# intel/oim

Hardware: AMD Instinct MI355X
Metric: 4KiB_randread_IOPS (higher is better)
Workload: dtype uint8

## Files before the change

### native/src/gpu.hip

```cpp

#include <hip/hip_runtime.h>
#include <pthread.h>
#include <sched.h>
#include <unistd.h>
#include <stdlib.h>

#include <algorithm>
#include <atomic>
#include <chrono>
#include <condition_variable>
#include <cstring>
#include <deque>
#include <functional>
#include <map>
#include <mutex>
#include <random>
#include <set>
#include <stdexcept>
#include <thread>
#include <utility>
#include <vector>

#include "hipstore/crc32c.h"
#include "hipstore/engine.h"
// ... 187 lines not shown
       w += gridDim.x) {
    const unsigned long long word = bitmap[w];
    const uint64_t g0 = w * 64;
    unsigned long long inside = word;
    if (g0 < win.g_begin) inside &= ~0ull << (win.g_begin - g0);
    if (win.g_end - g0 < 64) inside &= (1ull << (win.g_end - g0)) - 1;
    uint32_t bits = __builtin_amdgcn_readfirstlane(static_cast<uint32_t>(
        (inside >> (wave * kDiffGranulesPerWave)) & 0xFFFFu));
    if (bits == 0) continue;
    const uint32_t rank0 =
        __builtin_amdgcn_readfirstlane(rank_before_word[w]) - win.first_rank;
    while (bits != 0) {
      const uint32_t bit = wave * kDiffGranulesPerWave +
                           static_cast<uint32_t>(__builtin_ctz(bits));
      bits &= bits - 1;
      const uint32_t slot =
          rank0 + static_cast<uint32_t>(__popcll(word & ((1ull << bit) - 1)));
      if (slot >= win.count) break;
      uint4* __restrict__ pg = reinterpret_cast<uint4*>(
          bdev_base + (g0 + bit) * granule_bytes);
      uint4* __restrict__ ps = reinterpret_cast<uint4*>(
          dense + static_cast<uint64_t>(slot) * granule_bytes);
      if (kPack) {
#pragma unroll 4
        for (uint32_t i = lane; i < n16; i += 64) ps[i] = pg[i];
      } else {
#pragma unroll 4
        for (uint32_t i = lane; i < n16; i += 64) pg[i] = ps[i];
      }
    }
  }
}

__global__ __launch_bounds__(kWavesPerWg * 64) void k_pack_marked(
    const uint8_t* __restrict__ src, uint8_t* __restrict__ dense,
    const unsigned long long* __restrict__ bitmap,
    const uint32_t* __restrict__ rank_before_word, MarkedWindow win,
    uint32_t granule_bytes) {
  marked_window_walk<true>(const_cast<uint8_t*>(src), dense, bitmap,
                           rank_before_word, win, granule_bytes);
}

__global__ __launch_bounds__(kWavesPerWg * 64) void k_unpack_marked(
    uint8_t* __restrict__ dst, const uint8_t* __restrict__ dense,
    const unsigned long long* __restrict__ bitmap,
    const uint32_t* __restrict__ rank_before_word, MarkedWindow win,
    uint32_t granule_bytes) {
  marked_window_walk<false>(dst, const_cast<uint8_t*>(dense), bitmap,
                            rank_before_word, win, granule_bytes);
}


__device__ __forceinline__ unsigned long long wave_bcast_u64(
    unsigned long long v) {
  int lo = __shfl(static_cast<int>(v & 0xFFFFFFFFu), 0);
  int hi = __shfl(static_cast<int>(v >> 32), 0);
  return (static_cast<unsigned long long>(static_cast<uint32_t>(hi)) << 32) |
         static_cast<uint32_t>(lo);
}

__device__ __forceinline__ unsigned long long claim_bounded(
    unsigned long long* counter, unsigned long long c,
    unsigned long long kt, uint32_t lane) {
  while (c < kt) {
    unsigned long long witnessed = 0;
    if (lane == 0) {
      witnessed = atomicCAS(counter, c, c + 1);
    }
    witnessed = wave_bcast_u64(witnessed);
    if (witnessed == c) return c;
    c = witnessed;
  }
  return ~0ull;
}

struct PersistentCtl {
  const BlockDesc* sq;
  volatile unsigned long long* sq_tail;
  volatile unsigned long long* cq;
  volatile uint32_t* stop;
  unsigned long long* claim_counter;
  unsigned long long* known_tail;
  uint32_t* exit_flag;
  uint32_t ring_mask;
  uint32_t idle_spins;
};

__global__ __launch_bounds__(64) void k_persistent_copy(PersistentCtl ctl) {
  __shared__ __attribute__((aligned(16))) uint8_t lds_raw[kTileBytes];
  const uint32_t lane = threadIdx.x & 63;
  float4* lds = reinterpret_cast<float4*>(lds_raw);

  if (blockIdx.x == 0) {
    if (lane != 0) return;
    unsigned long long known = __hip_atomic_load(
        ctl.known_tail, __ATOMIC_RELAXED, __HIP_MEMORY_SCOPE_AGENT);
    uint32_t spins = 0;
    while (true) {
      unsigned long long tail = __hip_atomic_load(
          const_cast<const unsigned long long*>(ctl.sq_tail),
          __ATOMIC_ACQUIRE, __HIP_MEMORY_SCOPE_SYSTEM);
      if (tail > known) {
        known = tail;
        __hip_atomic_store(ctl.known_tail, known, __ATOMIC_RELEASE,
                           __HIP_MEMORY_SCOPE_AGENT);
        spins = 0;
      }
      if (__hip_atomic_load(const_cast<const uint32_t*>(ctl.stop),
                            __ATOMIC_RELAXED,
                            __HIP_MEMORY_SCOPE_SYSTEM) != 0 ||
          ++spins > ctl.idle_spins) {
        __hip_atomic_store(ctl.exit_flag, 1u, __ATOMIC_RELEASE,
                           __HIP_MEMORY_SCOPE_AGENT);
        return;
      }
      __builtin_amdgcn_s_sleep(8);
    }
  }

  while (true) {
    const unsigned long long kt = __hip_atomic_load(
        ctl.known_tail, __ATOMIC_RELAXED, __HIP_MEMORY_SCOPE_AGENT);
    const unsigned long long c = __hip_atomic_load(
        ctl.claim_counter, __ATOMIC_RELAXED, __HIP_MEMORY_SCOPE_AGENT);
    const unsigned long long claim =
        claim_bounded(ctl.claim_counter, c, kt, lane);
    if (claim == ~0ull) {
      if (__hip_atomic_load(ctl.exit_flag, __ATOMIC_RELAXED,
                            __HIP_MEMORY_SCOPE_AGENT) != 0) {
        return;
      }
      __builtin_amdgcn_s_sleep(16);
      continue;
    }
    const volatile unsigned long long* vd =
        reinterpret_cast<const volatile unsigned long long*>(
            &ctl.sq[claim & ctl.ring_mask]);
    const unsigned long long w0 = vd[0];
    const unsigned long long w1 = vd[1];
    const unsigned long long w2 = vd[2];
    BlockDesc d;
    d.src = reinterpret_cast<const uint8_t*>(w0);
    d.dst = reinterpret_cast<uint8_t*>(w1);
    d.bytes = static_cast<uint32_t>(w2 & 0xFFFFFFFFu);
    d.fill = static_cast<uint32_t>(w2 >> 32);
    const uint32_t n8 = d.bytes >> 3;
    unsigned long long* lds64 = reinterpret_cast<unsigned long long*>(lds);
    if (d.src != nullptr) {
      const unsigned long long* __restrict__ src =
          reinterpret_cast<const unsigned long long*>(d.src);
#pragma unroll 4
      for (uint32_t i = lane; i < n8; i += 64) {
        lds64[i] = __hip_atomic_load(src + i, __ATOMIC_RELAXED,
                                     __HIP_MEMORY_SCOPE_AGENT);
      }
    } else {
      const uint32_t b = d.fill & 0xFF;
      const uint32_t word = b | (b << 8) | (b << 16) | (b << 24);
      const unsigned long long v =
          word | (static_cast<unsigned long long>(word) << 32);
      for (uint32_t i = lane; i < n8; i += 64) lds64[i] = v;
    }
    unsigned long long* __restrict__ dst =
        reinterpret_cast<unsigned long long*>(d.dst);
#pragma unroll 4
    for (uint32_t i = lane; i < n8; i += 64) dst[i] = lds64[i];
    if (lane == 0) {
      __hip_atomic_store(&ctl.cq[claim & ctl.ring_mask], claim + 1,
                         __ATOMIC_RELEASE, __HIP_MEMORY_SCOPE_SYSTEM);
    }
  }
}

__global__ void k_init_ctl(unsigned long long* dst, unsigned long long a,
                           unsigned long long b, unsigned long long c) {
  if (threadIdx.x == 0) {
    dst[0] = a;
    dst[1] = b;
    dst[2] = c;
  }
}

std::atomic<uint64_t> g_pers_launches{0};
std::atomic<uint64_t> g_pers_relaunches{0};
std::atomic<uint64_t> g_pers_stall_queries{0};


struct SharedSlot {
  const BlockDesc* sq;
  volatile unsigned long long* sq_tail;
  volatile unsigned long long* cq;
  unsigned long long claim;
  unsigned long long known_tail;
  unsigned long long ring_mask_active;
};
static_assert(sizeof(SharedSlot) == 48, "8-byte atom layout");

constexpr uint32_t kSharedSlots = 64;

struct SharedCtl {
  SharedSlot* slots;
  volatile uint32_t* stop;
  uint32_t* exit_flag;
  uint32_t idle_spins;
};

__device__ __forceinline__ unsigned long long slot_ld(
    SharedSlot* slot, int word) {
  return __hip_atomic_load(
      reinterpret_cast<unsigned long long*>(slot) + word, __ATOMIC_RELAXED,
      __HIP_MEMORY_SCOPE_AGENT);
}

__device__ __forceinline__ void slot_st(SharedSlot* slot, int word,
                                        unsigned long long value) {
  __hip_atomic_store(reinterpret_cast<unsigned long long*>(slot) + word,
                     value, __ATOMIC_RELEASE, __HIP_MEMORY_SCOPE_AGENT);
}

__global__ __launch_bounds__(64) void k_shared_service(SharedCtl ctl) {
  __shared__ __attribute__((aligned(16))) uint8_t lds_raw[kTileBytes];
  const uint32_t lane = threadIdx.x & 63;
  float4* lds = reinterpret_cast<float4*>(lds_raw);

  if (blockIdx.x == 0) {
    SharedSlot* slot = &ctl.slots[lane];
    unsigned long long known = 0;
    uint32_t spins = 0;
    while (true) {
      bool advanced = false;
      if (slot_ld(slot, 5) >> 32) {
        volatile unsigned long long* tail_ptr =
            reinterpret_cast<volatile unsigned long long*>(slot_ld(slot, 1));
        const unsigned long long tail = __hip_atomic_load(
            const_cast<const unsigned long long*>(tail_ptr),
            __ATOMIC_ACQUIRE, __HIP_MEMORY_SCOPE_SYSTEM);
        if (tail > known) {
          known = tail;
          slot_st(slot, 4, known);
          advanced = true;
        }
      } else {
        known = 0;
      }
      const bool stop_now =
          lane == 0 &&
          __hip_atomic_load(const_cast<const uint32_t*>(ctl.stop),
                            __ATOMIC_RELAXED,
                            __HIP_MEMORY_SCOPE_SYSTEM) != 0;
      if (__any(advanced)) spins = 0;
      if (__any(stop_now) || ++spins > ctl.idle_spins) {
        if (lane == 0) {
          __hip_atomic_store(ctl.exit_flag, 1u, __ATOMIC_RELEASE,
                             __HIP_MEMORY_SCOPE_AGENT);
        }
        return;
      }
      __builtin_amdgcn_s_sleep(8);
    }
  }

  const uint32_t start = blockIdx.x;
  while (true) {
    bool progress = false;
    for (uint32_t i = 0; i < kSharedSlots; ++i) {
      SharedSlot* slot = &ctl.slots[(start + i) % kSharedSlots];
      const unsigned long long ma = slot_ld(slot, 5);
      if (!(ma >> 32)) continue;
// ... 108 lines not shown
    unsigned long long tail =
        ctl.use_atomics
            ? __hip_atomic_load(
                  const_cast<const unsigned long long*>(ctl.sq_tail),
                  __ATOMIC_ACQUIRE, __HIP_MEMORY_SCOPE_SYSTEM)
            : *ctl.sq_tail;
    if (tail != 0) {
      __hip_atomic_store(ctl.relay, tail, __ATOMIC_RELEASE,
                         __HIP_MEMORY_SCOPE_AGENT);
      if (ctl.do_fence) __threadfence_system();
      __hip_atomic_store(&ctl.cq[0], tail, __ATOMIC_RELEASE,
                         __HIP_MEMORY_SCOPE_SYSTEM);
      return;
    }
    __builtin_amdgcn_s_sleep(8);
  }
}

int g_device_count = -1;

struct HwQueueEnvInit {
  HwQueueEnvInit() {
    if (getenv("HIPSTORE_NO_HWQ_INIT") == nullptr) {
      setenv("GPU_MAX_HW_QUEUES", "24", 0);
    }
  }
};
HwQueueEnvInit g_hw_queue_env_init;

int device_count_cached() {
  static std::once_flag once;
  std::call_once(once, [] {
    int n = 0;
    if (hipGetDeviceCount(&n) != hipSuccess) n = 0;
    g_device_count = n;
  });
  return g_device_count;
}

double env_seconds(const char* name, double fallback) {
  const char* env = getenv(name);
  if (env == nullptr) return fallback;
  const double v = atof(env);
  return v > 0 ? v : fallback;
}

double sync_io_timeout_s() {
  static const double s = env_seconds("HIPSTORE_SYNC_TIMEOUT_S", 30.0);
  return s;
}

double teardown_timeout_s() {
  static const double s = env_seconds("HIPSTORE_TEARDOWN_TIMEOUT_S", 10.0);
  return s;
}

bool stream_drain(hipStream_t stream, double seconds) {
  const auto deadline = std::chrono::steady_clock::now() +
                        std::chrono::duration<double>(seconds);
  while (true) {
    if (hipStreamQuery(stream) != hipErrorNotReady) return true;
    if (std::chrono::steady_clock::now() > deadline) return false;
    std::this_thread::sleep_for(std::chrono::microseconds(200));
  }
}

void dump_engine_stats(const char* why) {
  fprintf(stderr,
          "[hipstore] %s: persistent-engine stats: launches=%llu "
          "relaunches=%llu stall_queries=%llu\n",
          why,
          static_cast<unsigned long long>(g_pers_launches.load()),
          static_cast<unsigned long long>(g_pers_relaunches.load()),
          static_cast<unsigned long long>(g_pers_stall_queries.load()));
}

}

uint64_t persistent_stat(int which) {
  switch (which) {
    case 0: return g_pers_launches.load();
    case 1: return g_pers_relaunches.load();
    case 2: return g_pers_stall_queries.load();
    default: return 0;
  }
}

bool gpu_available() { return device_count_cached() > 0; }
int gpu_device_count() { return device_count_cached(); }

std::string gpu_pci_address(int device) {
  char bus_id[32] = {0};
  if (hipDeviceGetPCIBusId(bus_id, sizeof(bus_id), device) != hipSuccess) {
    return "";
  }
  std::string s(bus_id);
  std::transform(s.begin(), s.end(), s.begin(), ::tolower);
  return s;
}

std::pair<uint64_t, uint64_t> hbm_info(int device) {
  if (!gpu_available() || device < 0 || device >= gpu_device_count()) {
    return {0, 0};
  }
  if (hipSetDevice(device) != hipSuccess) return {0, 0};
  size_t free_bytes = 0;
  size_t total_bytes = 0;
  if (hipMemGetInfo(&free_bytes, &total_bytes) != hipSuccess) return {0, 0};
  return {total_bytes, free_bytes};
}

void* alloc_pinned(size_t bytes) {
  if (!gpu_available()) return malloc(bytes);
  void* p = nullptr;
  HIP_CHECK(hipHostMalloc(&p, bytes, hipHostMallocMapped));
  return p;
}

void free_pinned(void* ptr) {
  if (ptr == nullptr) return;
  if (!gpu_available()) {
    free(ptr);
    return;
  }
  (void)hipHostFree(ptr);
}


namespace {

template <typename T>
T* device_view(T* host_ptr) {
  void* dev = nullptr;
  HIP_CHECK(hipHostGetDevicePointer(&dev, const_cast<void*>(
      reinterpret_cast<const void*>(host_ptr)), 0));
  return reinterpret_cast<T*>(dev);
}

class HbmChannelBase : public IoChannel {
 public:
  virtual void enqueue(IoRequest req, int status) = 0;
  virtual int poll() = 0;
  virtual const char* kind_name() const = 0;
};

inline HbmChannelBase* hbm_channel(IoChannel* ch) {
  return static_cast<HbmChannelBase*>(ch);
}

uint8_t* buf_device(uint8_t* host) {
  void* dev = nullptr;
  hipError_t err = hipHostGetDevicePointer(&dev, host, 0);
  if (err != hipSuccess) {
    throw std::runtime_error(
        "hipstore: I/O buffer is not pinned host memory (use alloc_pinned)");
  }
  return static_cast<uint8_t*>(dev);
}

inline uint32_t tile_count(uint64_t length) {
  return static_cast<uint32_t>((length + kTileBytes - 1) / kTileBytes);
}

void fill_desc(BlockDesc& d, const IoRequest& req, uint8_t* base,
               uint64_t done, uint32_t bytes) {
  if (req.op == IoOp::kRead) {
    d.src = base + req.offset + done;
// ... 258 lines not shown

 private:
  struct IoState {
    IoCompletion cb;
    uint32_t remaining;
    int status;
  };

  bool has_capacity(uint32_t tiles) const {
    return tail_ - completed_ + tiles <= kRing;
  }

  void drain_pending() {
    while (!pending_.empty()) {
      IoRequest& req = pending_.front();
      const uint32_t tiles = tile_count(req.length);
      if (!has_capacity(tiles)) return;
      auto* state = new IoState{std::move(req.on_complete), tiles, kIoOk};
      uint64_t done = 0;
      uint64_t t = tail_;
      while (done < req.length) {
        const uint32_t bytes = static_cast<uint32_t>(
            std::min<uint64_t>(kTileBytes, req.length - done));
        fill_desc(sq_[t % kRing], req, base_, done, bytes);
        desc_io_[t % kRing] = state;
        ++t;
        done += bytes;
      }
      tail_ = t;
      __atomic_store_n(const_cast<unsigned long long*>(sq_tail_), tail_,
                       __ATOMIC_RELEASE);
      pending_.pop_front();
    }
  }

  uint8_t* base_;
  std::vector<IoState*> desc_io_;
  std::deque<IoRequest> pending_;
  std::deque<std::pair<uint64_t, IoCompletion>> flushes_;
  std::vector<std::pair<IoCompletion, int>> immediate_;
};

inline std::atomic<int> g_per_queue_channels[64];
inline int per_queue_channel_cap() {
  static const int cap = [] {
    const char* env = getenv("HIPSTORE_PERQ_CAP");
    return env ? atoi(env) : 18;
  }();
  return cap;
}

inline bool fallback_is_shared() {
  static const bool shared = [] {
    const char* env = getenv("HIPSTORE_FALLBACK");
    return env == nullptr || strcmp(env, "batched") != 0;
  }();
  return shared;
}

class HbmPersistentChannel : public ServiceRingChannel {
 public:
  static constexpr uint32_t kIdleSpins = 500000;

  static uint32_t workers() {
    static uint32_t w = [] {
      const char* env = getenv("HIPSTORE_PERSISTENT_WORKERS");
      int v = env ? atoi(env) : 16;
      return static_cast<uint32_t>(std::min(std::max(v, 1), 64));
    }();
    return w;
  }

  HbmPersistentChannel(int device, uint8_t* base)
      : ServiceRingChannel(base), device_(device) {
    HIP_CHECK(hipSetDevice(device));
    HIP_CHECK(hipStreamCreateWithFlags(&stream_, hipStreamNonBlocking));
    alloc_rings();
    void* p_stop = nullptr;
    HIP_CHECK(hipHostMalloc(&p_stop, 4, hipHostMallocMapped));
    stop_ = static_cast<volatile uint32_t*>(p_stop);
    *stop_ = 0;
    HIP_CHECK(hipMalloc(reinterpret_cast<void**>(&claim_ctr_), 24));
    HIP_CHECK(hipMemset(claim_ctr_, 0, 24));
    HIP_CHECK(hipStreamSynchronize(nullptr));
    launch();
  }

  ~HbmPersistentChannel() override {
    g_per_queue_channels[device_].fetch_sub(1, std::memory_order_relaxed);
    __atomic_store_n(const_cast<uint32_t*>(stop_), 1u, __ATOMIC_RELEASE);
    if (!stream_drain(stream_, teardown_timeout_s())) {
      dump_engine_stats(
          "persistent-channel teardown timeout; leaking rings");
      return;
    }
    free_rings();
    (void)hipHostFree(const_cast<uint32_t*>(stop_));
    (void)hipFree(claim_ctr_);
    (void)hipStreamDestroy(stream_);
    delete_unfired();
  }

  const char* kind_name() const override { return "persistent"; }

 private:
  void on_stall() override {
    g_pers_stall_queries.fetch_add(1, std::memory_order_relaxed);
    if (hipStreamQuery(stream_) == hipSuccess) {
      g_pers_relaunches.fetch_add(1, std::memory_order_relaxed);
      launch();
    }
    debug_dump_state();
  }

  void launch() {
    g_pers_launches.fetch_add(1, std::memory_order_relaxed);
    (void)hipSetDevice(device_);
    static const bool use_memcpy = [] {
      const char* env = getenv("HIPSTORE_LAUNCH_INIT");
      return env != nullptr && strcmp(env, "memcpy") == 0;
    }();
    if (use_memcpy) {
      const unsigned long long init[3] = {completed_, completed_, 0};
      HIP_CHECK(hipMemcpyAsync(claim_ctr_, init, 24, hipMemcpyHostToDevice,
                               stream_));
    } else {
      hipLaunchKernelGGL(k_init_ctl, dim3(1), dim3(1), 0, stream_,
                         claim_ctr_, completed_, completed_, 0ull);
    }
    PersistentCtl ctl;
    ctl.sq = device_view(sq_);
    ctl.sq_tail = device_view(const_cast<unsigned long long*>(sq_tail_));
    ctl.cq = device_view(const_cast<unsigned long long*>(cq_));
    ctl.stop = device_view(const_cast<uint32_t*>(stop_));
    ctl.claim_counter = claim_ctr_;
    ctl.known_tail = claim_ctr_ + 1;
    ctl.exit_flag = reinterpret_cast<uint32_t*>(claim_ctr_ + 2);
    ctl.ring_mask = kRing - 1;
    ctl.idle_spins = kIdleSpins;
    hipLaunchKernelGGL(k_persistent_copy, dim3(workers() + 1), dim3(64), 0,
                       stream_, ctl);
    const hipError_t err = hipGetLastError();
    if (err != hipSuccess) {
      fprintf(stderr, "[hipstore] persistent service launch failed: %s\n",
              hipGetErrorString(err));
    }
    last_progress_ = std::chrono::steady_clock::now();
  }

  void debug_dump_state() {
    static const bool debug = getenv("HIPSTORE_DEBUG") != nullptr;
    if (!debug) return;
    const auto now = std::chrono::steady_clock::now();
    if (now - dbg_last_ < std::chrono::seconds(1)) return;
    dbg_last_ = now;
    if (dbg_stream_ == nullptr) {
      if (hipStreamCreateWithFlags(&dbg_stream_, hipStreamNonBlocking) !=
          hipSuccess) {
        return;
      }
    }
    unsigned long long words[3] = {0, 0, 0};
    (void)hipMemcpyAsync(words, claim_ctr_, 24, hipMemcpyDeviceToHost,
                         dbg_stream_);
    (void)hipStreamSynchronize(dbg_stream_);
    fprintf(stderr,
            "[hipstore-dbg] perq tail=%llu done=%llu sq_tail=%llu "
            "dev_claim=%llu dev_known=%llu dev_exit=%llu busy=%d\n",
            static_cast<unsigned long long>(tail_),
            static_cast<unsigned long long>(completed_), *sq_tail_,
            words[0], words[1], words[2],
            hipStreamQuery(stream_) == hipErrorNotReady);
  }

  std::chrono::steady_clock::time_point dbg_last_{};
  hipStream_t dbg_stream_ = nullptr;

  int device_;
  hipStream_t stream_ = nullptr;
  volatile uint32_t* stop_ = nullptr;
  unsigned long long* claim_ctr_ = nullptr;
};

class SharedService {
 public:
  static constexpr uint32_t kIdleSpins = 500000;

  static std::shared_ptr<SharedService>& instance(int device) {
    static std::mutex mutex;
    static std::map<int, std::shared_ptr<SharedService>> services;
    std::lock_guard<std::mutex> lock(mutex);
    auto& service = services[device];
    if (!service) service = std::make_shared<SharedService>(device);
    return service;
  }

  explicit SharedService(int device) : device_(device) {
    dbg("svc:setdev");
    HIP_CHECK(hipSetDevice(device));
    HIP_CHECK(hipStreamCreateWithFlags(&stream_, hipStreamNonBlocking));
    HIP_CHECK(hipStreamCreateWithFlags(&config_stream_, hipStreamNonBlocking));
    dbg("svc:malloc");
    HIP_CHECK(hipMalloc(reinterpret_cast<void**>(&slots_dev_),
                        kSharedSlots * sizeof(SharedSlot) + 8));
    dbg("svc:memset");
    HIP_CHECK(hipMemset(slots_dev_, 0, kSharedSlots * sizeof(SharedSlot) + 8));
    dbg("svc:nullsync");
    HIP_CHECK(hipStreamSynchronize(nullptr));
    dbg("svc:hostmalloc");
    exit_flag_dev_ = reinterpret_cast<uint32_t*>(slots_dev_ + kSharedSlots);
    void* p_stop = nullptr;
    HIP_CHECK(hipHostMalloc(&p_stop, 4, hipHostMallocMapped));
    stop_ = static_cast<volatile uint32_t*>(p_stop);
    *stop_ = 0;
    memset(mirror_, 0, sizeof(mirror_));
    memset(used_, 0, sizeof(used_));
    memset(prefix_, 0, sizeof(prefix_));
    HIP_CHECK(hipMemsetAsync(exit_flag_dev_, 0, 4, stream_));
    HIP_CHECK(hipMemsetAsync(exit_flag_dev_, 0, 4, config_stream_));
    HIP_CHECK(hipStreamSynchronize(stream_));
    HIP_CHECK(hipStreamSynchronize(config_stream_));
    dbg("svc:ctor-done");
  }

  static void dbg(const char* what) {
    if (getenv("HIPSTORE_DEBUG") != nullptr) {
      fprintf(stderr, "[hipstore-dbg] %s\n", what);
    }
  }


  int attach(const BlockDesc* sq_dev, unsigned long long* tail_dev,
             unsigned long long* cq_dev, uint32_t ring_mask) {
    std::lock_guard<std::mutex> lock(mutex_);
    for (uint32_t i = 0; i < kSharedSlots; ++i) {
      if (used_[i]) continue;
      used_[i] = true;
      prefix_[i] = 0;
      SharedSlot& m = mirror_[i];
      m.sq = sq_dev;
      m.sq_tail = tail_dev;
      m.cq = cq_dev;
      m.claim = 0;
      m.known_tail = 0;
      m.ring_mask_active = ring_mask;
      (void)hipSetDevice(device_);
      dbg("attach:copy");
      HIP_CHECK(hipMemcpyAsync(&slots_dev_[i], &m, 40, hipMemcpyHostToDevice,
                               config_stream_));
      m.ring_mask_active = ring_mask | (1ull << 32);
      HIP_CHECK(hipMemcpyAsync(
          reinterpret_cast<unsigned long long*>(&slots_dev_[i]) + 5,
          &m.ring_mask_active, 8, hipMemcpyHostToDevice, config_stream_));
      dbg("attach:sync");
      HIP_CHECK(hipStreamSynchronize(config_stream_));
      dbg("attach:launch");
      ensure_running_locked(true);
      dbg("attach:done");
      return static_cast<int>(i);
    }
    throw std::runtime_error("shared service: no free ring slots (64 max)");
  }

  void detach(int slot) {
// ... 1719 lines not shown
  std::this_thread::sleep_for(std::chrono::milliseconds(250));
  r["hb_host_early"] =
      static_cast<long long>(__atomic_load_n(hb, __ATOMIC_ACQUIRE));
  unsigned long long hb_dev_early = 0;
  (void)hipMemcpyAsync(&hb_dev_early, dev_words, 8, hipMemcpyDeviceToHost,
                       util);
  (void)hipStreamSynchronize(util);
  r["hb_dev_early"] = static_cast<long long>(hb_dev_early);
  __atomic_store_n(tail, 1ull, __ATOMIC_RELEASE);
  r["cq0_ms"] = -1;
  r["cq1_ms"] = -1;
  while (clock::now() - t0 < std::chrono::seconds(5)) {
    if (r["cq0_ms"] < 0 && __atomic_load_n(&cq[0], __ATOMIC_ACQUIRE) != 0) {
      r["cq0_ms"] = std::chrono::duration_cast<std::chrono::milliseconds>(
                        clock::now() - t0).count();
    }
    if (r["cq1_ms"] < 0 && __atomic_load_n(&cq[1], __ATOMIC_ACQUIRE) != 0) {
      r["cq1_ms"] = std::chrono::duration_cast<std::chrono::milliseconds>(
                        clock::now() - t0).count();
    }
    if (r["cq0_ms"] >= 0 && r["cq1_ms"] >= 0) break;
    std::this_thread::sleep_for(std::chrono::milliseconds(2));
  }
  r["hb_host_final"] =
      static_cast<long long>(__atomic_load_n(hb, __ATOMIC_ACQUIRE));
  unsigned long long dev_final[3] = {0, 0, 0};
  (void)hipMemcpyAsync(dev_final, dev_words, 24, hipMemcpyDeviceToHost,
                       util);
  (void)hipStreamSynchronize(util);
  r["hb_dev_final"] = static_cast<long long>(dev_final[0]);
  r["relay_final"] = static_cast<long long>(dev_final[1]);
  r["rmw_final"] = static_cast<long long>(dev_final[2]);
  const bool drained = stream_drain(stream, 10.0);
  r["stream_drained"] = drained;
  if (drained) {
    (void)hipHostFree(p_tail);
    (void)hipHostFree(p_hb);
    (void)hipHostFree(p_cq);
    (void)hipFree(dev_words);
    (void)hipStreamDestroy(stream);
  }
  (void)hipStreamDestroy(util);
  return r;
}


std::map<std::string, long long> persistent_kernel_probe(int device,
                                                         int variant) {
  constexpr uint32_t kProbeRing = 32768;
  std::map<std::string, long long> r;
  r["variant"] = variant;
  HIP_CHECK(hipSetDevice(device));
  hipStream_t stream = nullptr;
  hipStream_t util = nullptr;
  HIP_CHECK(hipStreamCreateWithFlags(&stream, hipStreamNonBlocking));
  HIP_CHECK(hipStreamCreateWithFlags(&util, hipStreamNonBlocking));
  BlockDesc* sq = nullptr;
  HIP_CHECK(hipHostMalloc(reinterpret_cast<void**>(&sq),
                          kProbeRing * sizeof(BlockDesc),
                          hipHostMallocMapped));
  void* p_tail = nullptr;
  void* p_cq = nullptr;
  void* p_stop = nullptr;
  void* p_buf = nullptr;
  HIP_CHECK(hipHostMalloc(&p_tail, 8, hipHostMallocMapped));
  HIP_CHECK(hipHostMalloc(&p_cq, kProbeRing * 8, hipHostMallocMapped));
  HIP_CHECK(hipHostMalloc(&p_stop, 4, hipHostMallocMapped));
  HIP_CHECK(hipHostMalloc(&p_buf, 8192, hipHostMallocMapped));
  auto* tail = static_cast<volatile unsigned long long*>(p_tail);
  auto* cq = static_cast<volatile unsigned long long*>(p_cq);
  auto* stop = static_cast<volatile uint32_t*>(p_stop);
  auto* buf = static_cast<uint8_t*>(p_buf);
  *tail = 0;
  *stop = 0;
  memset(const_cast<unsigned long long*>(cq), 0, kProbeRing * 8);
  memset(buf, 0x5A, 4096);
  memset(buf + 4096, 0, 4096);
  uint8_t* hbm = nullptr;
  HIP_CHECK(hipMalloc(reinterpret_cast<void**>(&hbm), 8192));
  HIP_CHECK(hipMemset(hbm, 0xA7, 8192));
  unsigned long long* claim_ctr = nullptr;
  HIP_CHECK(hipMalloc(reinterpret_cast<void**>(&claim_ctr), 24));
  HIP_CHECK(hipMemset(claim_ctr, 0, 24));
  HIP_CHECK(hipStreamSynchronize(nullptr));
  PersistentCtl ctl;
  ctl.sq = device_view(sq);
  ctl.sq_tail = device_view(const_cast<unsigned long long*>(tail));
  ctl.cq = device_view(const_cast<unsigned long long*>(cq));
  ctl.stop = device_view(const_cast<uint32_t*>(stop));
  ctl.claim_counter = claim_ctr;
  ctl.known_tail = claim_ctr + 1;
  ctl.exit_flag = reinterpret_cast<uint32_t*>(claim_ctr + 2);
  ctl.ring_mask = kProbeRing - 1;
  ctl.idle_spins = 500000;
  hipLaunchKernelGGL(k_persistent_copy, dim3(17), dim3(64), 0, stream, ctl);
  r["launch_err"] = static_cast<long long>(hipGetLastError());
  uint8_t* buf_dev = device_view(buf);
  BlockDesc& d = sq[0];
  switch (variant) {
    case 0:
      d.src = buf_dev;
      d.dst = buf_dev + 4096;
      d.bytes = 64;
      break;
    case 1:
      d.src = buf_dev;
      d.dst = hbm;
      d.bytes = 4096;
      break;
    default:
      d.src = hbm;
      d.dst = buf_dev + 4096;
      d.bytes = 4096;
      break;
  }
  d.fill = 0;
  __atomic_store_n(tail, 1ull, __ATOMIC_RELEASE);
  using clock = std::chrono::steady_clock;
  const auto t0 = clock::now();
  r["cq_ms"] = -1;
  while (clock::now() - t0 < std::chrono::seconds(4)) {
    if (__atomic_load_n(&cq[0], __ATOMIC_ACQUIRE) == 1) {
      r["cq_ms"] = std::chrono::duration_cast<std::chrono::milliseconds>(
                       clock::now() - t0).count();
      break;
    }
    std::this_thread::sleep_for(std::chrono::milliseconds(2));
  }
  unsigned long long words[3] = {0, 0, 0};
  (void)hipMemcpyAsync(words, claim_ctr, 24, hipMemcpyDeviceToHost, util);
  (void)hipStreamSynchronize(util);
  r["dev_claim"] = static_cast<long long>(words[0]);
  r["dev_known"] = static_cast<long long>(words[1]);
  r["dev_exit"] = static_cast<long long>(words[2]);
  r["data_ok"] = variant == 0   ? memcmp(buf, buf + 4096, 64) == 0
                 : variant == 2 ? buf[4096] == 0xA7 && buf[8191] == 0xA7
                                : -1;
  __atomic_store_n(stop, 1u, __ATOMIC_RELEASE);
  const bool drained = stream_drain(stream, 8.0);
  r["stream_drained"] = drained;
  if (drained) {
    (void)hipHostFree(sq);
    (void)hipHostFree(p_tail);
    (void)hipHostFree(p_cq);
    (void)hipHostFree(p_stop);
    (void)hipHostFree(p_buf);
    (void)hipFree(hbm);
    (void)hipFree(claim_ctr);
    (void)hipStreamDestroy(stream);
  }
  (void)hipStreamDestroy(util);
  return r;
}


}
```

### native/src/pybind.cpp

```cpp

#include <pybind11/functional.h>
#include <pybind11/pybind11.h>
#include <pybind11/stl.h>

#include <cstring>
#include <optional>
#include <stdexcept>

#include "hipstore/bdev.h"
#include "hipstore/composite.h"
#include "hipstore/crc32c.h"
#include "hipstore/delta.h"
#include "hipstore/engine.h"
#include "hipstore/nvmf.h"
#include "hipstore/rados.h"
#include "hipstore/vhost_master.h"

namespace py = pybind11;
using namespace hipstore;

namespace {

py::bytes bdev_read_py(Bdev& bdev, uint64_t offset, uint64_t length) {
  void* bounce = alloc_pinned(length);
// ... 485 lines not shown
                                bool overwrite) {
    DeltaInfo info;
    std::string error;
    int status;
    {
      py::gil_scoped_release release;
      status = bdev_export_delta(src.get(), base ? base->get() : nullptr,
                                 path, granule.value_or(0), overwrite, &info,
                                 &error);
    }
    if (status != kIoOk) throw_delta("bdev_export_delta", status, error);
    return delta_info_to_dict(info);
  }, py::arg("src"), py::arg("path"), py::arg("base") = py::none(),
     py::arg("granule") = py::none(), py::arg("overwrite") = false,
     "Write the granules of src that differ from base (every granule "
     "without a base) to a hipstore delta file");

  m.def("bdev_import_delta", [](BdevPtr dst, const std::string& path,
                                bool dry_run) {
    DeltaInfo info;
    std::string error;
    int status;
    {
      py::gil_scoped_release release;
      status = bdev_import_delta(dst.get(), path, dry_run, &info, &error);
    }
    if (status != kIoOk) throw_delta("bdev_import_delta", status, error);
    return delta_info_to_dict(info);
  }, py::arg("dst"), py::arg("path"), py::arg("dry_run") = false,
     "Apply a hipstore delta file to dst; dry_run checks everything and "
     "writes nothing");

  m.def("delta_file_info", [](const std::string& path) {
    DeltaInfo info;
    std::string error;
    const int status = delta_file_info(path, &info, &error);
    if (status != kIoOk) throw_delta("delta_file_info", status, error);
    return delta_info_to_dict(info);
  }, py::arg("path"), "Header fields of a delta file, after its structural checks");

  m.def("replica_scrub", [](BdevPtr bdev, bool repair, uint32_t granule,
                            uint32_t max_report) {
    ScrubResult r;
    {
      py::gil_scoped_release release;
      r = replicated_scrub(bdev.get(), repair, granule, max_report);
    }
    if (r.status != kIoOk) {
      throw std::runtime_error("replica_scrub failed: status " +
                               std::to_string(r.status));
    }
    py::list replicas;
    for (const ScrubReplica& rep : r.replicas) {
      py::dict d;
      d["child"] = rep.child;
      d["granules"] = rep.granules;
      d["mismatched"] = rep.mismatched;
      d["repaired"] = rep.repaired;
      d["first_mismatches"] = rep.first_mismatches;
      replicas.append(d);
    }
    py::dict out;
    out["granule"] = r.granule;
    out["replicas"] = replicas;
    return out;
  }, py::arg("bdev"), py::arg("repair") = false, py::arg("granule") = 0,
     py::arg("max_report") = 16,
     "Compare every replica of a replicated bdev with child 0; with "
     "repair, overwrite mismatching granules from it (refused while the "
     "bdev is claimed)");

  m.def("persistent_probe", &persistent_probe, py::arg("device") = 0,
        py::arg("flags") = 1,
        py::call_guard<py::gil_scoped_release>());
  m.def("persistent_kernel_probe", &persistent_kernel_probe,
        py::arg("device") = 0, py::arg("variant") = 0,
        py::call_guard<py::gil_scoped_release>());

  m.def("persistent_stats", [] {
    py::dict d;
    d["launches"] = hipstore::persistent_stat(0);
    d["relaunches"] = hipstore::persistent_stat(1);
    d["stall_queries"] = hipstore::persistent_stat(2);
    return d;
  });

  m.def("crc32c_combine", &crc32c_combine, py::arg("crc1"), py::arg("crc2"),
        py::arg("len2"));

  m.def("crc32c_table", [](py::buffer data, uint32_t init) {
    py::buffer_info info = data.request();
    return crc32c_table(init, info.ptr,
                        static_cast<size_t>(info.size) * info.itemsize);
  }, py::arg("data"), py::arg("init") = 0);
  m.def("crc32c", [](py::buffer data, uint32_t init) {
    py::buffer_info info = data.request();
    return crc32c_sw(init, info.ptr, static_cast<size_t>(info.size) * info.itemsize);
  }, py::arg("data"), py::arg("init") = 0);

  m.def("crc32c_gpu_blocks", [](BdevPtr bdev, uint64_t offset, uint32_t block,
                                uint32_t count) {
    std::vector<uint32_t> out(count);
    {
      py::gil_scoped_release release;
      crc32c_hbm_blocks(bdev.get(), offset, block, count, out.data());
    }
    return out;
  }, py::arg("bdev"), py::arg("offset"), py::arg("block"), py::arg("count"),
     "CRC32C of `count` consecutive `block`-byte blocks of an HBM bdev, "
     "computed on-GPU");

  m.def("crc32c_gpu_range", [](BdevPtr bdev, uint64_t offset,
                               uint64_t length) {
    py::gil_scoped_release release;
    return crc32c_hbm_range(bdev.get(), offset, length);
  }, py::arg("bdev"), py::arg("offset"), py::arg("length"),
     "CRC32C of one range: per-4 KiB block CRCs folded with "
     "crc32c_combine (the digest ladder of the NVMe-oF and rados paths)");
}
```

Measured before the change: 10.85 million.

## Mirror submission descriptors into device memory and copy tiles via buffer loads

The leader wave now reads newly submitted descriptors from host-mapped SQ memory cooperatively and copies them into a device-resident mirror. Workers then read descriptors from HBM at agent scope instead of issuing volatile system-scope loads over the bus. The per-IO copy drops the LDS staging and uses 128-bit raw buffer loads and stores held in registers. An optional phase-clock instrumentation variant, off by default, is added as a template parameter. The change adds leader-side work and a dependency on the mirror being published before known_tail.

```diff
diff --git a/native/src/gpu.hip b/native/src/gpu.hip
--- a/native/src/gpu.hip
+++ b/native/src/gpu.hip
@@ -293,42 +293,190 @@
   unsigned long long* claim_counter;
   unsigned long long* known_tail;
   uint32_t* exit_flag;
+  unsigned long long* mirror;
   uint32_t ring_mask;
   uint32_t idle_spins;
+  unsigned long long* stats;
 };
 
+enum PersStat : uint32_t {
+  kPersStatClaim = 0,
+  kPersStatDesc,
+  kPersStatLoad,
+  kPersStatStore,
+  kPersStatIdle,
+  kPersStatIos,
+  kPersStatLeaderTicks,
+  kPersStatLeaderIters,
+  kPersStatWords
+};
+constexpr uint32_t kPhaseFlushIos = 256;
+
+template <bool kOn>
+struct PhaseClock {
+  unsigned long long t = 0;
+  unsigned long long acc[kPersStatIos] = {};
+  uint32_t ios = 0;
+  __device__ __forceinline__ void start() {
+    if constexpr (kOn) t = wall_clock64();
+  }
+  __device__ __forceinline__ void mark(uint32_t phase, bool drain = false) {
+    if constexpr (kOn) {
+      if (drain) asm volatile("s_waitcnt vmcnt(0) lgkmcnt(0)" ::: "memory");
+      const unsigned long long now = wall_clock64();
+      acc[phase] += now - t;
+      t = now;
+    }
+  }
+  __device__ __forceinline__ void served(unsigned long long* stats,
+                                         uint32_t lane) {
+    if constexpr (kOn) {
+      ++ios;
+      if (ios >= kPhaseFlushIos) flush(stats, lane);
+    }
+  }
+  __device__ __forceinline__ void flush(unsigned long long* stats,
+                                        uint32_t lane) {
+    if constexpr (kOn) {
+      if (lane == 0) {
+        for (uint32_t p = 0; p < kPersStatIos; ++p) {
+          atomicAdd(&stats[p], acc[p]);
+        }
+        atomicAdd(&stats[kPersStatIos],
+                  static_cast<unsigned long long>(ios));
+      }
+      for (uint32_t p = 0; p < kPersStatIos; ++p) acc[p] = 0;
+      ios = 0;
+    }
+  }
+};
+
+typedef uint32_t u32x4 __attribute__((ext_vector_type(4)));
+constexpr uint32_t kTileRounds = kTileBytes / (64 * 16);
+constexpr int kBufferAuxSc1 = 16;
+
+__device__ __forceinline__ __amdgpu_buffer_rsrc_t tile_rsrc(
+    const uint8_t* base, uint32_t bytes) {
+  const unsigned long long addr = reinterpret_cast<unsigned long long>(base);
+  const uint32_t lo =
+      __builtin_amdgcn_readfirstlane(static_cast<uint32_t>(addr));
+  const uint32_t hi =
+      __builtin_amdgcn_readfirstlane(static_cast<uint32_t>(addr >> 32));
+  const uint32_t size = __builtin_amdgcn_readfirstlane(
+      bytes < kTileBytes ? bytes : kTileBytes);
+  return __builtin_amdgcn_make_buffer_rsrc(
+      reinterpret_cast<void*>((static_cast<unsigned long long>(hi) << 32) |
+                              lo),
+      0, size, 0x00020000 );
+}
+
+__device__ __forceinline__ void tile_load(const BlockDesc& d, uint32_t lane,
+                                          u32x4 (&v)[kTileRounds]) {
+  if (d.src != nullptr) {
+    const __amdgpu_buffer_rsrc_t rsrc = tile_rsrc(d.src, d.bytes);
+#pragma unroll
+    for (uint32_t r = 0; r < kTileRounds; ++r) {
+      v[r] = __builtin_amdgcn_raw_buffer_load_b128(
+          rsrc, lane * 16 + r * 1024, 0, kBufferAuxSc1);
+    }
+  } else {
+    const uint32_t b = d.fill & 0xFF;
+    const uint32_t word = b | (b << 8) | (b << 16) | (b << 24);
+#pragma unroll
+    for (uint32_t r = 0; r < kTileRounds; ++r) {
+      v[r] = u32x4{word, word, word, word};
+    }
+  }
+}
+
+__device__ __forceinline__ void tile_store(const BlockDesc& d, uint32_t lane,
+                                           const u32x4 (&v)[kTileRounds]) {
+  const __amdgpu_buffer_rsrc_t rsrc = tile_rsrc(d.dst, d.bytes);
+#pragma unroll
+  for (uint32_t r = 0; r < kTileRounds; ++r) {
+    __builtin_amdgcn_raw_buffer_store_b128(v[r], rsrc, lane * 16 + r * 1024,
+                                           0, 0);
+  }
+}
+
+template <bool kPhaseClock>
 __global__ __launch_bounds__(64) void k_persistent_copy(PersistentCtl ctl) {
-  __shared__ __attribute__((aligned(16))) uint8_t lds_raw[kTileBytes];
   const uint32_t lane = threadIdx.x & 63;
-  float4* lds = reinterpret_cast<float4*>(lds_raw);
 
   if (blockIdx.x == 0) {
-    if (lane != 0) return;
     unsigned long long known = __hip_atomic_load(
         ctl.known_tail, __ATOMIC_RELAXED, __HIP_MEMORY_SCOPE_AGENT);
+    const unsigned long long* sq_words =
+        reinterpret_cast<const unsigned long long*>(ctl.sq);
     uint32_t spins = 0;
+    unsigned long long lead_t0 = 0;
+    unsigned long long lead_iters = 0;
+    if constexpr (kPhaseClock) lead_t0 = wall_clock64();
     while (true) {
-      unsigned long long tail = __hip_atomic_load(
-          const_cast<const unsigned long long*>(ctl.sq_tail),
-          __ATOMIC_ACQUIRE, __HIP_MEMORY_SCOPE_SYSTEM);
-      if (tail > known) {
-        known = tail;
-        __hip_atomic_store(ctl.known_tail, known, __ATOMIC_RELEASE,
-                           __HIP_MEMORY_SCOPE_AGENT);
+      if constexpr (kPhaseClock) ++lead_iters;
+      unsigned long long tail = 0;
+      uint32_t stop = 0;
+      if (lane == 0) {
+        tail = __hip_atomic_load(
+            const_cast<const unsigned long long*>(ctl.sq_tail),
+            __ATOMIC_RELAXED, __HIP_MEMORY_SCOPE_SYSTEM);
+        stop = __hip_atomic_load(const_cast<const uint32_t*>(ctl.stop),
+                                 __ATOMIC_RELAXED, __HIP_MEMORY_SCOPE_SYSTEM);
+      }
+      tail = wave_bcast_u64(tail);
+      stop = static_cast<uint32_t>(__shfl(static_cast<int>(stop), 0));
+      while (known < tail) {
+        const uint32_t n = static_cast<uint32_t>(
+            tail - known < 64 ? tail - known : 64);
+        unsigned long long v[3];
+        uint32_t pos[3];
+#pragma unroll
+        for (uint32_t k = 0; k < 3; ++k) {
+          const uint32_t w = lane + 64 * k;
+          pos[k] = (static_cast<uint32_t>(known + w / 3) & ctl.ring_mask) * 3 +
+                   w % 3;
+          v[k] = 0;
+          if (w < n * 3) {
+            v[k] = __hip_atomic_load(sq_words + pos[k], __ATOMIC_RELAXED,
+                                     __HIP_MEMORY_SCOPE_SYSTEM);
+          }
+        }
+#pragma unroll
+        for (uint32_t k = 0; k < 3; ++k) {
+          if (lane + 64 * k < n * 3) {
+            __hip_atomic_store(ctl.mirror + pos[k], v[k], __ATOMIC_RELAXED,
+                               __HIP_MEMORY_SCOPE_AGENT);
+          }
+        }
+        asm volatile("s_waitcnt vmcnt(0)" ::: "memory");
+        known += n;
+        if (lane == 0) {
+          __hip_atomic_store(ctl.known_tail, known, __ATOMIC_RELEASE,
+                             __HIP_MEMORY_SCOPE_AGENT);
+        }
         spins = 0;
       }
-      if (__hip_atomic_load(const_cast<const uint32_t*>(ctl.stop),
-                            __ATOMIC_RELAXED,
-                            __HIP_MEMORY_SCOPE_SYSTEM) != 0 ||
-          ++spins > ctl.idle_spins) {
-        __hip_atomic_store(ctl.exit_flag, 1u, __ATOMIC_RELEASE,
-                           __HIP_MEMORY_SCOPE_AGENT);
+      if (stop != 0 || ++spins > ctl.idle_spins) {
+        if (lane == 0) {
+          __hip_atomic_store(ctl.exit_flag, 1u, __ATOMIC_RELEASE,
+                             __HIP_MEMORY_SCOPE_AGENT);
+        }
         return;
       }
       __builtin_amdgcn_s_sleep(8);
-    }
-  }
-
+      if constexpr (kPhaseClock) {
+        if (lane == 0 && (lead_iters & 1023) == 0) {
+          const unsigned long long now = wall_clock64();
+          atomicAdd(&ctl.stats[kPersStatLeaderTicks], now - lead_t0);
+          atomicAdd(&ctl.stats[kPersStatLeaderIters], 1024ull);
+          lead_t0 = now;
+        }
+      }
+    }
+  }
+
+  PhaseClock<kPhaseClock> clk;
+  clk.start();
   while (true) {
     const unsigned long long kt = __hip_atomic_load(
         ctl.known_tail, __ATOMIC_RELAXED, __HIP_MEMORY_SCOPE_AGENT);
@@ -339,47 +487,38 @@
     if (claim == ~0ull) {
       if (__hip_atomic_load(ctl.exit_flag, __ATOMIC_RELAXED,
                             __HIP_MEMORY_SCOPE_AGENT) != 0) {
+        clk.flush(ctl.stats, lane);
         return;
       }
       __builtin_amdgcn_s_sleep(16);
+      clk.mark(kPersStatIdle);
       continue;
     }
-    const volatile unsigned long long* vd =
-        reinterpret_cast<const volatile unsigned long long*>(
-            &ctl.sq[claim & ctl.ring_mask]);
-    const unsigned long long w0 = vd[0];
-    const unsigned long long w1 = vd[1];
-    const unsigned long long w2 = vd[2];
+    clk.mark(kPersStatClaim);
+    const unsigned long long* vd =
+        ctl.mirror + static_cast<uint32_t>(claim & ctl.ring_mask) * 3;
+    const unsigned long long w0 =
+        __hip_atomic_load(vd + 0, __ATOMIC_RELAXED, __HIP_MEMORY_SCOPE_AGENT);
+    const unsigned long long w1 =
+        __hip_atomic_load(vd + 1, __ATOMIC_RELAXED, __HIP_MEMORY_SCOPE_AGENT);
+    const unsigned long long w2 =
+        __hip_atomic_load(vd + 2, __ATOMIC_RELAXED, __HIP_MEMORY_SCOPE_AGENT);
     BlockDesc d;
     d.src = reinterpret_cast<const uint8_t*>(w0);
     d.dst = reinterpret_cast<uint8_t*>(w1);
     d.bytes = static_cast<uint32_t>(w2 & 0xFFFFFFFFu);
     d.fill = static_cast<uint32_t>(w2 >> 32);
-    const uint32_t n8 = d.bytes >> 3;
-    unsigned long long* lds64 = reinterpret_cast<unsigned long long*>(lds);
-    if (d.src != nullptr) {
-      const unsigned long long* __restrict__ src =
-          reinterpret_cast<const unsigned long long*>(d.src);
-#pragma unroll 4
-      for (uint32_t i = lane; i < n8; i += 64) {
-        lds64[i] = __hip_atomic_load(src + i, __ATOMIC_RELAXED,
-                                     __HIP_MEMORY_SCOPE_AGENT);
-      }
-    } else {
-      const uint32_t b = d.fill & 0xFF;
-      const uint32_t word = b | (b << 8) | (b << 16) | (b << 24);
-      const unsigned long long v =
-          word | (static_cast<unsigned long long>(word) << 32);
-      for (uint32_t i = lane; i < n8; i += 64) lds64[i] = v;
-    }
-    unsigned long long* __restrict__ dst =
-        reinterpret_cast<unsigned long long*>(d.dst);
-#pragma unroll 4
-    for (uint32_t i = lane; i < n8; i += 64) dst[i] = lds64[i];
+    clk.mark(kPersStatDesc, true);
+    u32x4 tile[kTileRounds];
+    tile_load(d, lane, tile);
+    clk.mark(kPersStatLoad, true);
+    tile_store(d, lane, tile);
     if (lane == 0) {
       __hip_atomic_store(&ctl.cq[claim & ctl.ring_mask], claim + 1,
                          __ATOMIC_RELEASE, __HIP_MEMORY_SCOPE_SYSTEM);
     }
+    clk.mark(kPersStatStore, true);
+    clk.served(ctl.stats, lane);
   }
 }
 
@@ -395,6 +534,63 @@
 std::atomic<uint64_t> g_pers_launches{0};
 std::atomic<uint64_t> g_pers_relaunches{0};
 std::atomic<uint64_t> g_pers_stall_queries{0};
+
+std::mutex g_pers_dev_stats_mutex;
+unsigned long long* g_pers_dev_stats[64] = {};
+
+unsigned long long* pers_dev_stats(int device) {
+  std::lock_guard<std::mutex> lock(g_pers_dev_stats_mutex);
+  if (g_pers_dev_stats[device] == nullptr) {
+    void* p = nullptr;
+    HIP_CHECK(hipMalloc(&p, kPersStatWords * 8));
+    HIP_CHECK(hipMemset(p, 0, kPersStatWords * 8));
+    HIP_CHECK(hipStreamSynchronize(nullptr));
+    g_pers_dev_stats[device] = static_cast<unsigned long long*>(p);
+  }
+  return g_pers_dev_stats[device];
+}
+
+uint64_t pers_dev_stat(uint32_t word) {
+  std::lock_guard<std::mutex> lock(g_pers_dev_stats_mutex);
+  uint64_t sum = 0;
+  for (int device = 0; device < 64; ++device) {
+    if (g_pers_dev_stats[device] == nullptr) continue;
+    static hipStream_t util[64] = {};
+    if (hipSetDevice(device) != hipSuccess) continue;
+    if (util[device] == nullptr &&
+        hipStreamCreateWithFlags(&util[device], hipStreamNonBlocking) !=
+            hipSuccess) {
+      continue;
+    }
+    unsigned long long v = 0;
+    if (hipMemcpyAsync(&v, g_pers_dev_stats[device] + word, 8,
+                       hipMemcpyDeviceToHost, util[device]) == hipSuccess &&
+        hipStreamSynchronize(util[device]) == hipSuccess) {
+      sum += v;
+    }
+  }
+  return sum;
+}
+
+bool persistent_phase_clock() {
+  static const bool on = [] {
+    const char* env = getenv("HIPSTORE_PERSISTENT_PHASE_CLOCK");
+    return env != nullptr && atoi(env) != 0;
+  }();
+  return on;
+}
+
+void launch_persistent_kernel(PersistentCtl ctl, int device, uint32_t workers,
+                              hipStream_t stream) {
+  ctl.stats = pers_dev_stats(device);
+  if (persistent_phase_clock()) {
+    hipLaunchKernelGGL(k_persistent_copy<true>, dim3(workers + 1), dim3(64),
+                       0, stream, ctl);
+  } else {
+    hipLaunchKernelGGL(k_persistent_copy<false>, dim3(workers + 1), dim3(64),
+                       0, stream, ctl);
+  }
+}
 
 
 struct SharedSlot {
@@ -669,7 +865,12 @@
     case 0: return g_pers_launches.load();
     case 1: return g_pers_relaunches.load();
     case 2: return g_pers_stall_queries.load();
-    default: return 0;
+    case 3: return persistent_phase_clock() ? 1 : 0;
+    default:
+      if (which >= 16 && which < 16 + static_cast<int>(kPersStatWords)) {
+        return pers_dev_stat(static_cast<uint32_t>(which - 16));
+      }
+      return 0;
   }
 }
 
@@ -1094,6 +1295,9 @@
     *stop_ = 0;
     HIP_CHECK(hipMalloc(reinterpret_cast<void**>(&claim_ctr_), 24));
     HIP_CHECK(hipMemset(claim_ctr_, 0, 24));
+    HIP_CHECK(hipMalloc(reinterpret_cast<void**>(&mirror_),
+                        kRing * sizeof(BlockDesc)));
+    HIP_CHECK(hipMemset(mirror_, 0, kRing * sizeof(BlockDesc)));
     HIP_CHECK(hipStreamSynchronize(nullptr));
     launch();
   }
@@ -1109,6 +1313,7 @@
     free_rings();
     (void)hipHostFree(const_cast<uint32_t*>(stop_));
     (void)hipFree(claim_ctr_);
+    (void)hipFree(mirror_);
     (void)hipStreamDestroy(stream_);
     delete_unfired();
   }
@@ -1148,10 +1353,10 @@
     ctl.claim_counter = claim_ctr_;
     ctl.known_tail = claim_ctr_ + 1;
     ctl.exit_flag = reinterpret_cast<uint32_t*>(claim_ctr_ + 2);
+    ctl.mirror = mirror_;
     ctl.ring_mask = kRing - 1;
     ctl.idle_spins = kIdleSpins;
-    hipLaunchKernelGGL(k_persistent_copy, dim3(workers() + 1), dim3(64), 0,
-                       stream_, ctl);
+    launch_persistent_kernel(ctl, device_, workers(), stream_);
     const hipError_t err = hipGetLastError();
     if (err != hipSuccess) {
       fprintf(stderr, "[hipstore] persistent service launch failed: %s\n",
@@ -1175,14 +1380,19 @@
     unsigned long long words[3] = {0, 0, 0};
     (void)hipMemcpyAsync(words, claim_ctr_, 24, hipMemcpyDeviceToHost,
                          dbg_stream_);
+    unsigned long long staged[3] = {0, 0, 0};
+    (void)hipMemcpyAsync(staged, mirror_ + (completed_ % kRing) * 3, 24,
+                         hipMemcpyDeviceToHost, dbg_stream_);
     (void)hipStreamSynchronize(dbg_stream_);
     fprintf(stderr,
             "[hipstore-dbg] perq tail=%llu done=%llu sq_tail=%llu "
-            "dev_claim=%llu dev_known=%llu dev_exit=%llu busy=%d\n",
+            "dev_claim=%llu dev_known=%llu dev_exit=%llu busy=%d "
+            "mirror[done]={src=%#llx dst=%#llx bytes|fill=%#llx}\n",
             static_cast<unsigned long long>(tail_),
             static_cast<unsigned long long>(completed_), *sq_tail_,
             words[0], words[1], words[2],
-            hipStreamQuery(stream_) == hipErrorNotReady);
+            hipStreamQuery(stream_) == hipErrorNotReady,
+            staged[0], staged[1], staged[2]);
   }
 
   std::chrono::steady_clock::time_point dbg_last_{};
@@ -1192,6 +1402,7 @@
   hipStream_t stream_ = nullptr;
   volatile uint32_t* stop_ = nullptr;
   unsigned long long* claim_ctr_ = nullptr;
+  unsigned long long* mirror_ = nullptr;
 };
 
 class SharedService {
@@ -3077,6 +3288,10 @@
   unsigned long long* claim_ctr = nullptr;
   HIP_CHECK(hipMalloc(reinterpret_cast<void**>(&claim_ctr), 24));
   HIP_CHECK(hipMemset(claim_ctr, 0, 24));
+  unsigned long long* mirror = nullptr;
+  HIP_CHECK(hipMalloc(reinterpret_cast<void**>(&mirror),
+                      kProbeRing * sizeof(BlockDesc)));
+  HIP_CHECK(hipMemset(mirror, 0, kProbeRing * sizeof(BlockDesc)));
   HIP_CHECK(hipStreamSynchronize(nullptr));
   PersistentCtl ctl;
   ctl.sq = device_view(sq);
@@ -3086,9 +3301,10 @@
   ctl.claim_counter = claim_ctr;
   ctl.known_tail = claim_ctr + 1;
   ctl.exit_flag = reinterpret_cast<uint32_t*>(claim_ctr + 2);
+  ctl.mirror = mirror;
   ctl.ring_mask = kProbeRing - 1;
   ctl.idle_spins = 500000;
-  hipLaunchKernelGGL(k_persistent_copy, dim3(17), dim3(64), 0, stream, ctl);
+  launch_persistent_kernel(ctl, device, 16, stream);
   r["launch_err"] = static_cast<long long>(hipGetLastError());
   uint8_t* buf_dev = device_view(buf);
   BlockDesc& d = sq[0];
@@ -3142,6 +3358,7 @@
     (void)hipHostFree(p_buf);
     (void)hipFree(hbm);
     (void)hipFree(claim_ctr);
+    (void)hipFree(mirror);
     (void)hipStreamDestroy(stream);
   }
   (void)hipStreamDestroy(util);
diff --git a/native/src/pybind.cpp b/native/src/pybind.cpp
--- a/native/src/pybind.cpp
+++ b/native/src/pybind.cpp
@@ -591,6 +591,13 @@
     d["launches"] = hipstore::persistent_stat(0);
     d["relaunches"] = hipstore::persistent_stat(1);
     d["stall_queries"] = hipstore::persistent_stat(2);
+    d["phase_clock"] = hipstore::persistent_stat(3) != 0;
+    static const char* const kWords[] = {
+        "claim_ticks", "desc_ticks", "load_ticks", "store_ticks",
+        "idle_ticks", "phase_ios", "leader_ticks", "leader_iters"};
+    for (int w = 0; w < 8; ++w) {
+      d[kWords[w]] = hipstore::persistent_stat(16 + w);
+    }
     return d;
   });
 
```

Result: slower. 8.695 million (-19.9%).
